# OverLordGoldDragon/ssqueezepy

Hardware: AMD Instinct MI355X
Metric: ssq_cwt transforms/sec (N=160k, 300 scales, f32) (higher is better)
Workload: dtype f32; 1 GPU; ssq_cwt('gmw'), N=160000, 300 log scales (nv=32), float32, two-chirp+noise; algo=blockzoom+tiles, tile_kernel=float64 tile, unordered ds_add_f64, column pair per lane (tile3_kernel)

## Files before the change

include/ssq_hip.h:

```cpp
#ifndef SSQ_HIP_H
#define SSQ_HIP_H

#include <stdint.h>

#ifdef __cplusplus
extern "C" {
#endif

#define SSQ_F32 0
#define SSQ_F64 1

#define SSQ_GRID_LOG 0
#define SSQ_GRID_LOG_PIECEWISE 1
#define SSQ_GRID_LIN 2

#define SSQ_PAD_NONE (-1)
#define SSQ_PAD_ZERO 0
#define SSQ_PAD_REFLECT 1
#define SSQ_PAD_SYMMETRIC 2
#define SSQ_PAD_REPLICATE 3
#define SSQ_PAD_WRAP 4

int         ssq_version(void);
const char* ssq_build_sha(void);
// ... 145 lines not shown
    const int32_t* generic_rows;
    int64_t        n_generic;
} ssq_cwt_blocks_desc;

int  ssq_cwt_plan_set_blocks(ssq_cwt_plan* plan, const ssq_cwt_blocks_desc* desc);

typedef struct {
    int32_t        n_segs;
    const int32_t* segs;
    int32_t        n_steps;
    const int32_t* rows;
    const void*    wtab;
    int64_t        n_phases;
    const void*    tbank;
    int64_t        n_tbank;
    int32_t        n_irows;
    const int64_t* irows;
    int32_t        n_classes;
    const int64_t* classes;
    int64_t        u_total;
    int64_t        n_items_tile[5];
    int32_t        reserved;
} ssq_cwt_tiles_desc;

int  ssq_cwt_plan_set_tiles(ssq_cwt_plan* plan, const ssq_cwt_tiles_desc* desc);

int  ssq_cwt_plan_timing(ssq_cwt_plan* plan, int enable, double* stage_ms, int64_t* signals);

int  ssq_cwt_plan_group(const ssq_cwt_plan* plan);

int64_t ssq_cwt_plan_tiles_done(ssq_cwt_plan* plan, void* stream);
int  ssq_cwt_plan_tile_cols(const ssq_cwt_plan* plan);
int  ssq_cwt_plan_tile_kernel(const ssq_cwt_plan* plan);
int  ssq_cwt_plan_tile_counters(ssq_cwt_plan* plan, unsigned long long* out, int n, void* stream);

int  ssq_cwt_plan_set_bin_dump(ssq_cwt_plan* plan, unsigned short* kmap);

int  ssq_cwt_tile_rows_per_step(void);

int64_t ssq_cwt_plan_bytes(const ssq_cwt_plan* plan);
const char* ssq_cwt_plan_algo(const ssq_cwt_plan* plan);

typedef struct ssq_stft_plan ssq_stft_plan;

typedef struct {
    int      dtype;
    int      padtype;
    int64_t  n;
    int64_t  n_fft;
    int64_t  hop_len;
    int      modulated;
    const void* window;
    const void* diff_window;
    int64_t  max_batch;
} ssq_stft_desc;

int  ssq_stft_plan_create(ssq_stft_plan** plan, const ssq_stft_desc* desc);
void ssq_stft_plan_destroy(ssq_stft_plan* plan);
int  ssq_stft_plan_set_ssq(ssq_stft_plan* plan, const void* Sfs, int grid,
                           const double* params, const void* cst, int cst_f64,
                           int flipud, double gamma);
int  ssq_stft_plan_shape(const ssq_stft_plan* plan, int64_t* rows, int64_t* n_hops);
const char* ssq_stft_plan_algo(const ssq_stft_plan* plan);
int  ssq_stft_execute(ssq_stft_plan* plan, const void* x, int64_t batch, void* Sx,
                      void* dSx, void* Tx, void* w, void* stream);
int  ssq_stft_adjoint(ssq_stft_plan* plan, const void* gSx, const void* gdSx, void* gx,
// ... 7 lines not shown
```

ssqueezepy_amd/_cwt.py:

```python
import ctypes
import logging
import os
import numpy as np
import torch

from . import _lib
from ._lib import check, F32, F64, CwtDesc, CwtBlocksDesc, CwtTilesDesc
from . import algos
from ._bank import banded_bank, support_hull
from ._blocks import plan_blocks, L_MIN
from ._tiles import plan_tiles, RSUB as _tiles_rsub
from .padding import pad_geometry, PADTYPES
from .scales import process_scales, _process_fs_and_t
from .wavelets import Wavelet

WARN = lambda msg: logging.warning("WARNING: %s" % msg)

__all__ = ['cwt', 'cwt_higher_order', 'CwtPlan', 'get_cwt_plan', 'clear_plan_cache']

_TDT = {'float32': torch.float32, 'float64': torch.float64}
_CDT = {'float32': torch.complex64, 'float64': torch.complex128}


class CwtPlan():
# ... 137 lines not shown
        d.n_classes, d.classes = len(classes), classes.ctypes.data
        d.u_total = tp['u_total']
        d.reserved = _tiles_rsub
        for slot in range(5):
            d.n_items_tile[slot] = n_items_tile[slot]
        check(self.lib.ssq_cwt_plan_set_tiles(self._h, ctypes.byref(d)))
        self.tile_rows = int(tp['interp_rows'].sum())
        self.tile_plan = {k: tp[k] for k in ('lgR', 'interp_rows', 'classes')}

    def __del__(self):
        h = getattr(self, '_h', None)
        if h is not None and h.value:
            try:
                self.lib.ssq_cwt_plan_destroy(h)
            except Exception:
                pass
            self._h = None

    @property
    def algo(self):
        return self.lib.ssq_cwt_plan_algo(self._h).decode()

    def tiles_done(self):
        return int(self.lib.ssq_cwt_plan_tiles_done(self._h, algos.stream()))

    @property
    def tile_cols(self):
        return int(self.lib.ssq_cwt_plan_tile_cols(self._h))

    @property
    def tile_kernel(self):
        return int(self.lib.ssq_cwt_plan_tile_kernel(self._h))

    def set_bin_dump(self, kmap):
        if kmap is not None and (kmap.element_size() != 2 or kmap.numel() < self.max_batch * self.na * self.N
                                 or not kmap.is_contiguous()):
            raise ValueError("bin dump: a contiguous 2-byte tensor of max_batch * na * N elements is needed")
        check(self.lib.ssq_cwt_plan_set_bin_dump(self._h, kmap.data_ptr() if kmap is not None else None))
        self._kdump = kmap

    def tiles_per_signal(self, N):
        if not self.tile_cols:
            return 0
        lead = (self.n1 & 1) if self.tile_kernel == 3 else 0
        return -(-(int(N) + lead) // self.tile_cols)

    @property
    def device_bytes(self):
        return int(self.lib.ssq_cwt_plan_bytes(self._h))

    @property
    def group(self):
        return int(self.lib.ssq_cwt_plan_group(self._h))

    def timing(self, enable=-1):
        ms = (ctypes.c_double * 4)()
        n = ctypes.c_int64()
        check(self.lib.ssq_cwt_plan_timing(self._h, int(enable), ms, ctypes.byref(n)))
        return list(ms), int(n.value)

    def set_ssq(self, grid, params, const, flipud, gamma):
        const = np.asarray(const)
        if const.size != self.na:
            const = np.full(self.na, float(const)).astype(self.dtype)
        const = const.reshape(-1)
        c64 = int(self.dtype == 'float32' and const.dtype == np.float64)
# ... 263 lines not shown
```

ssqueezepy_amd/_lib.py:

```python
import ctypes
import os
from ctypes import (c_int, c_int64, c_double, c_void_p, c_char_p, POINTER,
                    Structure)

HERE = os.path.dirname(os.path.abspath(__file__))
LIB_PATH = os.environ.get('SSQ_HIP_LIB') or os.path.join(HERE, 'libssq_hip.so')

F32, F64 = 0, 1
GRID_LOG, GRID_LOG_PIECEWISE, GRID_LIN = 0, 1, 2
PAD = {None: -1, 'zero': 0, 'reflect': 1, 'symmetric': 2, 'replicate': 3,
       'wrap': 4}


class SsqError(RuntimeError):
    pass


class CwtDesc(Structure):
    _fields_ = [('dtype', c_int), ('padtype', c_int), ('n', c_int64),
                ('m', c_int64), ('n1', c_int64), ('na', c_int64),
                ('bank', c_void_p), ('band_off', c_void_p), ('band_lo', c_void_p),
                ('dt', c_double), ('row_scale', c_void_p), ('max_batch', c_int64),
                ('algo', c_int)]

# ... 71 lines not shown
    'ssq_colsum_adjoint': (c_int, [c_int, c_void_p, c_void_p, c_void_p, c_int64, c_int64,
                                   c_int64, c_void_p]),
    'ssq_band_colsum_batch': (c_int, [c_int, c_void_p, c_void_p, c_void_p, c_int, c_int64,
                                      c_void_p, c_int64, c_int64, c_int64, c_void_p]),
    'ssq_band_colsum_adjoint': (c_int, [c_int, c_void_p, c_void_p, c_void_p, c_int, c_int64,
                                        c_void_p, c_int64, c_int64, c_int64, c_void_p]),
    'ssq_ridge_energy': (c_int, [c_int, c_int, c_void_p, c_void_p, c_int64, c_int64, c_void_p]),
    'ssq_ridge_neglog': (c_int, [c_int, c_void_p, c_void_p, c_double, c_int64, c_int64, c_void_p]),
    'ssq_ridge_track': (c_int, [c_int, c_int, c_void_p, c_void_p, c_void_p, c_double, c_double,
                                c_int64, c_int64, c_void_p, c_void_p]),
    'ssq_ridge_clear': (c_int, [c_int, c_void_p, c_void_p, c_double, c_void_p, c_int64, c_int64,
                                c_void_p]),
    'ssq_ridge_neglog_batch': (c_int, [c_int, c_void_p, c_void_p, c_double, c_int64, c_int64, c_int64,
                                       c_void_p]),
    'ssq_ridge_track_batch': (c_int, [c_int, c_int, c_void_p, c_void_p, c_void_p, c_double, c_double,
                                      c_int64, c_int64, c_void_p, c_int64, c_void_p]),
    'ssq_ridge_clear_batch': (c_int, [c_int, c_void_p, c_void_p, c_double, c_void_p, c_int64, c_int64,
                                      c_int64, c_void_p]),
    'ssq_cwt_plan_create': (c_int, [POINTER(c_void_p), POINTER(CwtDesc)]),
    'ssq_cwt_plan_destroy': (None, [c_void_p]),
    'ssq_cwt_plan_set_ssq': (c_int, [c_void_p, c_int, POINTER(c_double), c_void_p,
                                     c_int, c_int, c_double]),
    'ssq_cwt_execute': (c_int, [c_void_p, c_void_p, c_int64, c_void_p, c_void_p,
                                c_void_p, c_void_p, c_int, c_void_p]),
    'ssq_cwt_plan_set_blocks': (c_int, [c_void_p, POINTER(CwtBlocksDesc)]),
    'ssq_cwt_plan_set_tiles': (c_int, [c_void_p, POINTER(CwtTilesDesc)]),
    'ssq_cwt_plan_timing': (c_int, [c_void_p, c_int, POINTER(c_double), POINTER(c_int64)]),
    'ssq_cwt_plan_group': (c_int, [c_void_p]),
    'ssq_cwt_plan_bytes': (c_int64, [c_void_p]),
    'ssq_cwt_plan_algo': (c_char_p, [c_void_p]),
    'ssq_cwt_plan_tiles_done': (c_int64, [c_void_p, c_void_p]),
    'ssq_cwt_plan_tile_cols': (c_int, [c_void_p]),
    'ssq_cwt_plan_tile_kernel': (c_int, [c_void_p]),
    'ssq_cwt_plan_tile_counters': (c_int, [c_void_p, c_void_p, c_int, c_void_p]),
    'ssq_cwt_plan_set_bin_dump': (c_int, [c_void_p, c_void_p]),
    'ssq_build_sha': (c_char_p, []),
    'ssq_cwt_tile_rows_per_step': (c_int, []),
    'ssq_stft_plan_create': (c_int, [POINTER(c_void_p), POINTER(StftDesc)]),
    'ssq_stft_plan_destroy': (None, [c_void_p]),
    'ssq_stft_plan_set_ssq': (c_int, [c_void_p, c_void_p, c_int, POINTER(c_double),
                                      c_void_p, c_int, c_int, c_double]),
    'ssq_stft_plan_shape': (c_int, [c_void_p, POINTER(c_int64), POINTER(c_int64)]),
    'ssq_stft_plan_algo': (c_char_p, [c_void_p]),
    'ssq_stft_execute': (c_int, [c_void_p, c_void_p, c_int64, c_void_p, c_void_p,
                                 c_void_p, c_void_p, c_void_p]),
    'ssq_stft_adjoint': (c_int, [c_void_p, c_void_p, c_void_p, c_void_p, c_int64, c_void_p]),
}

EXPORTS = tuple(_PROTOS)
_lib = None


ABI_VERSION = 107


def load(build_if_missing=True):
    global _lib
    if _lib is not None:
        return _lib
    if not os.path.isfile(LIB_PATH):
        if not build_if_missing:
            raise SsqError("libssq_hip.so not found at %s; run "
                           "`python -m ssqueezepy_amd.build`" % LIB_PATH)
        from .build import build
        build(verbose=False)
    try:
        lib = ctypes.CDLL(LIB_PATH)
    except OSError as e:
        raise SsqError("cannot load %s: %s. The ssqueezepy_amd compute path has no "
                       "CPU fallback; it needs the ROCm runtime (libamdhip64, "
                       "librocfft)." % (LIB_PATH, e))
    lib.ssq_version.restype, lib.ssq_version.argtypes = c_int, []
    if lib.ssq_version() < ABI_VERSION:
        raise SsqError("%s is an older build (ABI %d, this package needs %d); rebuild with "
                       "`python -m ssqueezepy_amd.build`"
                       % (LIB_PATH, lib.ssq_version(), ABI_VERSION))
    for name, (res, args) in _PROTOS.items():
        fn = getattr(lib, name)
        fn.restype = res
        fn.argtypes = args
    _lib = lib
    return lib


def check(rc):
    if rc != 0:
# ... 11 lines not shown
```

ssqueezepy_amd/csrc/ssq_cwt.hip:

```cpp
#include "ssq_common.h"
#include "ssq_fft.h"
#include "ssq_blocks.h"
#include "ssq_tiles.h"
#include <algorithm>
#include <map>
#include <string>
#include <vector>

namespace ssq {

#include "ssq_point_math.inl"

template <typename T>
__global__ __launch_bounds__(256) void bank_multiply_kernel(
    const T* __restrict__ xh,
    const T* __restrict__ bank, const int64_t* __restrict__ band_off,
    const int32_t* __restrict__ band_lo,
    T* __restrict__ prod,
    int64_t M, const int32_t* __restrict__ rowlist, int64_t row0, int nplanes, double h, T inv_dt) {
    const int64_t r = blockIdx.y;
    const int64_t i = rowlist[row0 + r];
    const int64_t lo = band_lo[i];
    const int64_t off = band_off[i];
    const int64_t len = band_off[i + 1] - off;
// ... 278 lines not shown
    if (stage_ms) for (int t = 0; t < 4; ++t) stage_ms[t] = pl->stage_ms[t];
    if (signals) *signals = pl->timed_signals;
    if (enable >= 0) {
        pl->timing = enable != 0;
        for (int t = 0; t < 4; ++t) pl->stage_ms[t] = 0;
        pl->timed_signals = 0;
    }
    return 0;
}

int ssq_cwt_plan_set_bin_dump(ssq_cwt_plan* pl, unsigned short* kmap) {
    SSQ_REQUIRE(pl, "ssq_cwt_plan_set_bin_dump: null plan");
    std::lock_guard<std::mutex> lock(pl->order.mu);
    pl->kdump = kmap;
    return 0;
}

int ssq_cwt_plan_group(const ssq_cwt_plan* pl) { return pl ? pl->group : 0; }
int ssq_cwt_tile_rows_per_step(void) { return ssq::tile_rows_per_step(); }
int64_t ssq_cwt_plan_tiles_done(ssq_cwt_plan* pl, void* stream) {
    if (!pl || !pl->tile) return 0;
    return pl->tile->tiles_done(as_stream(stream));
}
int ssq_cwt_plan_tile_cols(const ssq_cwt_plan* pl) { return (pl && pl->tile) ? pl->tile->tile_cols() : 0; }
int ssq_cwt_plan_tile_counters(ssq_cwt_plan* pl, unsigned long long* out, int n, void* stream) {
    SSQ_REQUIRE(pl && out && n >= 0 && n <= 512, "ssq_cwt_plan_tile_counters: bad arguments");
    memset(out, 0, (size_t)n * 8);
    if (!pl->tile || !pl->tile->counters) return 0;
    SSQ_CHECK_HIP(hipStreamSynchronize(as_stream(stream)));
    SSQ_CHECK_HIP(hipMemcpy(out, pl->tile->counters, (size_t)n * 8, hipMemcpyDeviceToHost));
    return 0;
}
int ssq_cwt_plan_tile_kernel(const ssq_cwt_plan* pl) { return (pl && pl->tile) ? pl->tile->tile_kernel() : 0; }
int64_t ssq_cwt_plan_bytes(const ssq_cwt_plan* pl) { return pl ? pl->bytes : 0; }
const char* ssq_cwt_plan_algo(const ssq_cwt_plan* pl) { return pl ? pl->algo.c_str() : ""; }

}

template <typename T>
static int cwt_execute_t(ssq_cwt_plan* pl, const void* x, int64_t batch, void* Wx, void* dWx,
                         void* Tx, void* w, int rpadded, hipStream_t stream) {
    const ssq_cwt_desc& d = pl->d;
    const int64_t M = d.m, N = d.n, na = d.na;
    const int64_t out_cols = rpadded ? M : N;
    const bool deriv = dWx || Tx || w;
    const int nplanes = deriv ? 2 : 1;
    const double h = (2.0 * 3.141592653589793) / (double)M;
    const T inv_dt = T(1) / (T)d.dt;
    if (pl->timing && pl->tev.size() < 2) {
        for (int t = 0; t < 2; ++t) { hipEvent_t e; SSQ_CHECK_HIP(hipEventCreate(&e)); pl->tev.push_back(e); }
    }
    if (pl->timing) (void)hipEventRecord(pl->tev[0], stream);

    const T* xsrc = (const T*)x;
    if (d.padtype != SSQ_PAD_NONE) {
        int rc = ssq_pad_signal(d.dtype, x, pl->xp, batch, N, d.n1, M - N - d.n1, d.padtype, stream);
        if (rc) return rc;
        xsrc = (const T*)pl->xp;
    } else {
        SSQ_CHECK_HIP(hipMemcpyAsync(pl->xp, x, (size_t)batch * M * sizeof(T), hipMemcpyDeviceToDevice, stream));
        xsrc = (const T*)pl->xp;
    }
    if (batch == d.max_batch) {
        int rc = pl->fwd.execute((void*)xsrc, pl->xh, stream);
        if (rc) return rc;
    } else {
// ... 172 lines not shown
```

ssqueezepy_amd/csrc/ssq_cwt_tiles.hip:

```cpp
#include "ssq_common.h"
#include "ssq_tiles.h"
#include <algorithm>
#include <cmath>

namespace ssq {

int tile_rows_per_step() { return TILE_G; }

struct ItemTable {
    int n = 0;
    std::vector<int32_t> rec;
    std::vector<int32_t> cls;
    std::vector<int32_t> woff;
    bool ok = true;
};
static ItemTable pack_items(const TileSeg* sg, int nsegs, const TileRow* rw, int nsteps, int64_t M, int64_t N, int rpi,
                            bool woff_in_record) {
    ItemTable t;
    t.n = nsteps * TILE_G / rpi;
    t.rec.assign((size_t)t.n * 8, 0); t.cls.assign((size_t)t.n, 0); t.woff.assign((size_t)t.n, 0);
    for (int i = 0; i < nsegs; ++i) {
        const int64_t L = (int64_t)M >> sg[i].lgR;
        if (sg[i].kind && (sg[i].wtab_off >= (woff_in_record ? 16384 : 65536) || sg[i].sig_stride % L)) t.ok = false;
        for (int s = 0; s < sg[i].nsteps * TILE_G / rpi; ++s) {
// ... 197 lines not shown
        if ((rc = up(&items2, t2.rec.data(), t2.rec.size() * 4))) return rc;
        if ((rc = up((void**)&wave_first2, waves.data(), waves.size() * 4))) return rc;
        tile3_ok = false;
        if (cols2 == 32) {
            ItemTable t3 = pack_items(sg, nsegs, rw, nsteps, M, N, 4, true);
            std::vector<int32_t> dealt;
            tile3_ok = deal_item_lists(t3, TILE3_NW, 0.45f, 0.65f, dealt, waves);
            n_items3 = t3.n;
            if ((rc = up(&items3, dealt.data(), dealt.size() * 4))) return rc;
            if ((rc = up((void**)&wave_first3, waves.data(), waves.size() * 4))) return rc;
            for (int i = 0; i < nsegs; ++i) if (sg[i].kind && sg[i].lgR < 2) tile3_ok = false;
        }
    }
    {
        const TileSeg* sg = reinterpret_cast<const TileSeg*>(d.segs);
        const float* src = reinterpret_cast<const float*>(d.wtab);
        std::vector<float> w((size_t)16 * d.n_phases, 0.f);
        std::vector<char> done((size_t)d.n_phases, 0);
        for (int i = 0; i < nsegs; ++i) {
            if (sg[i].kind != 1) continue;
            const int64_t R = (int64_t)1 << sg[i].lgR, o = sg[i].wtab_off;
            SSQ_REQUIRE(o >= 0 && o + R <= d.n_phases, "tile segment %d: weights outside the table", i);
            if (done[(size_t)o]) continue;
            done[(size_t)o] = 1;
            for (int64_t ph = 0; ph < R; ++ph)
                for (int t = 0; t < 4; ++t)
                    for (int k = 0; k < 4; ++k)
                        w[(size_t)(16 * o + (t * R + ph) * 4 + k)] = src[(size_t)(16 * (o + ph) + 4 * t + k)];
        }
        if ((rc = up(&wtab, w.data(), (size_t)64 * d.n_phases))) return rc;
    }
    if ((rc = up(&tbank, d.tbank, (size_t)4 * d.n_tbank))) return rc;
    cls.resize(d.n_classes);
    const bool own_fft = !(getenv("SSQ_DEBUG_TILE_FFT") && !strcmp(getenv("SSQ_DEBUG_TILE_FFT"), "rocfft"));
    int64_t y_entries = 0;
    for (int c = 0; c < d.n_classes; ++c) {
        cls[c] = {d.classes[4 * c], d.classes[4 * c + 1], d.classes[4 * c + 2], 0, 0, 0};
        SSQ_REQUIRE(cls[c].L >= 2 && (cls[c].L & (cls[c].L - 1)) == 0 && cls[c].nrows >= 1, "bad tile class %d", c);
        lmax = std::max(lmax, cls[c].L);
        int lg = 0;
        while (((int64_t)1 << lg) < cls[c].L) ++lg;
        if (own_fft && lg >= 13 && lg <= 22) {
            cls[c].B = 1 << ((lg + 1) / 2); cls[c].A = 1 << (lg / 2);
            y_entries += (int64_t)group * cls[c].nrows * cls[c].L;
        } else if (own_fft && lg >= 6 && lg <= 12) {
            cls[c].B = 1;
        }
    }
    std::vector<TileIRow> hi;
    hi.reserve((size_t)n_irows);
    for (int pass = 0; pass < 2; ++pass)
        for (int c = 0; c < d.n_classes; ++c) {
            if ((cls[c].A > 0 || cls[c].B > 0) != (pass == 0)) continue;
            if (pass == 1 && n_irows_fft == 0) first_irow_fft = (int)hi.size();
            cls[c].first = (int)hi.size();
            for (int r = 0; r < n_irows; ++r) {
                const int64_t* q = d.irows + 8 * r;
                if ((int)q[6] != c) continue;
                SSQ_REQUIRE(q[4] == cls[c].L && q[2] >= 1 && 2 * q[2] <= q[4]
                            && q[1] >= 0 && q[1] + q[2] <= M / 2 + 1 && q[5] >= 0 && q[5] + q[2] <= d.n_tbank
                            && q[7] >= 0 && q[7] < cls[c].nrows, "bad tile row %d", r);
                hi.push_back({(int32_t)q[0], (int32_t)q[1], (int32_t)q[2], (int32_t)q[3], (int32_t)q[4], (int32_t)q[5],
                              (int32_t)((int64_t)group * cls[c].upre + q[7] * cls[c].L), (int32_t)(cls[c].nrows * cls[c].L)});
            }
            SSQ_REQUIRE((int64_t)hi.size() - cls[c].first == cls[c].nrows, "tile class %d: %lld rows listed, %lld declared",
                        c, (long long)((int64_t)hi.size() - cls[c].first), (long long)cls[c].nrows);
            if (pass == 1) n_irows_fft += (int)cls[c].nrows;
        }
    SSQ_REQUIRE((int)hi.size() == n_irows, "tile rows of unknown classes");
    if ((rc = up((void**)&irows, hi.data(), sizeof(TileIRow) * n_irows))) return rc;
    if (own_fft) {
        SSQ_CHECK_HIP(hipMalloc(&Y, (size_t)8 * std::max<int64_t>(y_entries, 1))); bytes += 8 * y_entries;
        std::vector<float> tw;
        for (int s = 0; s < 7; ++s) {
            const int Lp = 64 << s;
            ftw_off[s] = (int64_t)tw.size() / 2;
            for (int q = 0; q < Lp; ++q) {
                const double a = 6.283185307179586 * (double)q / (double)Lp;
                tw.push_back((float)std::cos(a)); tw.push_back((float)std::sin(a));
            }
        }
        if ((rc = up(&ftw, tw.data(), tw.size() * 4))) return rc;
    }
    SSQ_CHECK_HIP(hipMalloc(&U, (size_t)8 * (group * u_total + 4 * lmax))); bytes += 8 * (group * u_total + 4 * lmax);
    SSQ_CHECK_HIP(hipMemset(U, 0, (size_t)8 * (group * u_total + 4 * lmax)));
    SSQ_CHECK_HIP(hipMalloc((void**)&counters, 4096));
    SSQ_CHECK_HIP(hipMemset(counters, 0, 4096));
    for (size_t c = 0; c < cls.size(); ++c) {
        FftPlan fp;
        if (!cls[c].A && !cls[c].B) {
            rc = fp.create(1, SSQ_F32, (size_t)cls[c].L, (size_t)(group * cls[c].nrows), 1.0);
            if (rc) return rc;
            bytes += (int64_t)fp.work_bytes;
        }
        ffts.push_back(fp);
    }
    for (int t = 0; t < 5; ++t) n_items_tile[t] = d.n_items_tile[t];
    SSQ_CHECK_HIP(hipStreamCreateWithFlags(&side, hipStreamNonBlocking));
    SSQ_CHECK_HIP(hipEventCreateWithFlags(&ev_fork, hipEventDisableTiming));
    SSQ_CHECK_HIP(hipEventCreateWithFlags(&ev_join, hipEventDisableTiming));
    return 0;
}

void TilePlan::destroy() {
    if (side) { (void)hipStreamSynchronize(side); (void)hipStreamDestroy(side); side = nullptr; }
// ... 36 lines not shown
        return run_ordered(sig, nsig, Wx, dWx, Tx, kidx, cst, cst0, sp, stream);
    default:
        set_error("na = %lld: no tile kernel can run in this mode (the executor asks usable() first)", (long long)na);
        return -1;
    }
}

TileWalkArgs TilePlan::walk_args(const void* items, const int32_t* waves, int sig, int nsig, float* Wx, float* dWx,
                                 float* Tx, const unsigned short* kidx, const void* cst, float cst0,
                                 const SsqParams& sp, unsigned short* kdump) const {
    TileWalkArgs A{};
    A.items = reinterpret_cast<const int*>(items); A.waves = reinterpret_cast<const int4*>(waves);
    A.wtab = (const float4*)wtab; A.U = (const float2*)U; A.cst = cst;
    A.Wx = (float2*)Wx; A.dWx = (float2*)dWx; A.Tx = (float2*)Tx; A.kidx = kidx; A.kdump = kdump;
    A.N = N; A.na = na; A.n1 = (int)n1; A.mmask = (int)(M - 1);
    A.lgM = 0; while (((int64_t)1 << A.lgM) < M) ++A.lgM;
    A.sig0 = sig; A.nsig = nsig; A.carry = 0; A.xcd = 0;
    A.inv_m = 1.0f / (float)M; A.theta_scale = (float)(6.283185307179586 / ((double)M * dt)); A.cst0 = cst0;
    A.counters = counters; A.gamma = sp.gamma;
    return A;
}

int TilePlan::walk_grid(int64_t ntx, int cols, int per_cu, TileWalkArgs& A) const {
    const int64_t cap = (int64_t)ncu * per_cu;
    const int64_t q = std::max<int64_t>(1, ((int64_t)1 << lgr_max2) / cols);
    const int64_t G = ntx <= cap ? ntx : std::max<int64_t>(q, cap / q * q);
    const char* ce = getenv("SSQ_DEBUG_TILE2_CARRY");
    A.carry = (!(ce && atoi(ce) == 0) && ntx > G && ntx % q == 0) ? 1 : 0;
    const char* xe = getenv("SSQ_DEBUG_TILE2_XCD");
    A.xcd = !(xe && atoi(xe) == 0) && G >= 16;
    return (int)G;
}

int64_t TilePlan::tiles_done(hipStream_t stream) {
    unsigned long long v = 0;
    if (!counters) return 0;
    if (hipStreamSynchronize(stream) != hipSuccess) return -1;
    if (hipMemcpy(&v, counters, 8, hipMemcpyDeviceToHost) != hipSuccess) return -1;
    return (int64_t)v;
}

}
```

ssqueezepy_amd/csrc/ssq_kernels.hip:

```cpp
#include "ssq_common.h"
#include <cstdlib>
#include <mutex>
#include <string>

namespace ssq {

static thread_local std::string g_last_error;

void set_error(const char* fmt, ...) {
    char buf[1024];
    va_list ap;
    va_start(ap, fmt);
    vsnprintf(buf, sizeof(buf), fmt, ap);
    va_end(ap);
    g_last_error = buf;
}

#include "ssq_point_math.inl"

template <typename T, bool CST64>
__device__ __forceinline__ void weighted_add(T& o_re, T& o_im, T c, T d, const void* cst, int64_t i) {
    if constexpr (CST64 && sizeof(T) == 4) {
        double w = ((const double*)cst)[i];
        o_re = (T)((double)o_re + (double)c * w);
// ... 604 lines not shown
        case SSQ_PAD_REPLICATE: return t < 0 ? 0 : n - 1;
        case SSQ_PAD_WRAP: { int64_t m = t % n; if (m < 0) m += n; return m; }
        default: return -1;
    }
}

template <typename T>
__global__ __launch_bounds__(256) void pad_kernel(const T* __restrict__ x, T* __restrict__ out,
                                                  int64_t n, int64_t n1, int64_t m, int padtype,
                                                  int64_t total) {
    for (int64_t t = (int64_t)blockIdx.x * blockDim.x + threadIdx.x; t < total;
         t += (int64_t)gridDim.x * blockDim.x) {
        int64_t b = t / m, p = t % m;
        int64_t s = pad_source(p - n1, n, padtype);
        out[t] = s < 0 ? T(0) : x[b * n + s];
    }
}

static inline unsigned stream_grid(int64_t total, int block = 256) {
    int64_t g = (total + block - 1) / block;
    const int64_t cap = 256 * 8 * 4;
    return (unsigned)(g < 1 ? 1 : (g > cap ? cap : g));
}

}

using namespace ssq;

extern "C" __attribute__((weak)) const char ssq_build_sha_value[] = "unknown";

extern "C" {

const char* ssq_build_sha(void) { return ssq_build_sha_value; }
int ssq_version(void) { return 107; }
const char* ssq_last_error(void) { return g_last_error.c_str(); }

int ssq_device_count(int* count) {
    SSQ_REQUIRE(count, "ssq_device_count: null pointer");
    SSQ_CHECK_HIP(hipGetDeviceCount(count));
    return 0;
}
int ssq_set_device(int device) { SSQ_CHECK_HIP(hipSetDevice(device)); return 0; }

int ssq_device_info(int device, char* name, int len, int* cus, int64_t* hbm_bytes) {
    hipDeviceProp_t prop;
    SSQ_CHECK_HIP(hipGetDeviceProperties(&prop, device));
    if (name && len > 0) { strncpy(name, prop.gcnArchName, len - 1); name[len - 1] = 0; }
    if (cus) *cus = prop.multiProcessorCount;
    if (hbm_bytes) *hbm_bytes = (int64_t)prop.totalGlobalMem;
    return 0;
}

int ssq_malloc(void** ptr, int64_t bytes) {
    SSQ_REQUIRE(ptr && bytes >= 0, "ssq_malloc: bad arguments");
    SSQ_CHECK_HIP(hipMalloc(ptr, (size_t)(bytes > 0 ? bytes : 1)));
    return 0;
}
int ssq_free(void* ptr) { SSQ_CHECK_HIP(hipFree(ptr)); return 0; }
int ssq_memcpy_h2d(void* dst, const void* src, int64_t bytes, void* stream) {
    SSQ_CHECK_HIP(hipMemcpyAsync(dst, src, (size_t)bytes, hipMemcpyHostToDevice, as_stream(stream)));
    return 0;
}
int ssq_memcpy_d2h(void* dst, const void* src, int64_t bytes, void* stream) {
    SSQ_CHECK_HIP(hipMemcpyAsync(dst, src, (size_t)bytes, hipMemcpyDeviceToHost, as_stream(stream)));
    return 0;
}
int ssq_memset(void* dst, int value, int64_t bytes, void* stream) {
// ... 151 lines not shown
```

ssqueezepy_amd/csrc/ssq_tile_fft.hip:

```cpp
#include "ssq_common.h"
#include "ssq_tiles.h"
#include "ssq_ldsfft.h"
#include <algorithm>
#include <cmath>

namespace ssq {

__global__ __launch_bounds__(256) void tile_spectra_kernel(const float2* __restrict__ xh_all,
                                                           int64_t xh_stride, int sig0,
                                                           const TileIRow* __restrict__ irows,
                                                           const float* __restrict__ tbank,
                                                           float2* __restrict__ U) {
    const TileIRow r = irows[blockIdx.y];
    const int s = blockIdx.z;
    const float2* xh = xh_all + (int64_t)(sig0 + s) * xh_stride;
    float2* u = U + r.ubase + (int64_t)s * r.sig_stride;
    const int half = r.L >> 1;
    for (int p = blockIdx.x * blockDim.x + threadIdx.x; p < r.L; p += gridDim.x * blockDim.x) {
        const int kk = p < half ? p : p - r.L;
        const int t = r.kc + kk - r.lo;
        float2 z = make_float2(0.f, 0.f);
        if (t >= 0 && t < r.K) {
            const float2 x = xh[r.lo + t];
            const float b = tbank[r.tb_off + t];
// ... 181 lines not shown
    for (int it = 0; it < PPT; ++it) {
        const int idx = tid + it * NT, q = idx & (L - 1), g = idx >> LGL;
        const int j = block * G + g;
        if (j < npairs) {
            const int jr = j % E.nrows, js = j / E.nrows;
            const TileIRow row = E.irows[jr];
            E.U[row.ubase + (int64_t)js * row.sig_stride + q] = buf[g * (L + 1) + q];
        }
    }
}

struct TileSmallArgs {
    TileFftArgs E[7];
    int first_block[8];
    int npairs[7], slot[7];
    int ncls;
};
__global__ __launch_bounds__(NT) void tilefft_small_kernel(TileSmallArgs A) {
    __shared__ c32 buf[D_POINTS + 64];
    int b = (int)blockIdx.x, c = 0;
    while (c + 1 < A.ncls && b >= A.first_block[c + 1]) ++c;
    b -= A.first_block[c];
    switch (A.slot[c]) {
        case 0: tilefft_small_body<64, 64, 8, 8, 1>(A.E[c], A.npairs[c], b, buf); break;
        case 1: tilefft_small_body<128, 32, 16, 8, 1>(A.E[c], A.npairs[c], b, buf); break;
        case 2: tilefft_small_body<256, 16, 16, 16, 1>(A.E[c], A.npairs[c], b, buf); break;
        case 3: tilefft_small_body<512, 8, 8, 8, 8>(A.E[c], A.npairs[c], b, buf); break;
        case 4: tilefft_small_body<1024, 4, 16, 8, 8>(A.E[c], A.npairs[c], b, buf); break;
        case 5: tilefft_small_body<2048, 2, 16, 16, 8>(A.E[c], A.npairs[c], b, buf); break;
        default: tilefft_small_body<4096, 1, 16, 16, 16>(A.E[c], A.npairs[c], b, buf); break;
    }
}

int TilePlan::spectra(int sig, int nsig, const void* xh_all, hipStream_t stream) {
    {
        TileSmallArgs S;
        S.ncls = 0; S.first_block[0] = 0;
        for (int want = 6; want >= 0; --want)
            for (size_t c = 0; c < cls.size() && S.ncls < 7; ++c) {
                if (cls[c].A || !cls[c].B) continue;
                int sl = 0;
                while ((64 << sl) < cls[c].L) ++sl;
                if (sl != want) continue;
                TileFftArgs& E = S.E[S.ncls];
                E.xh = (const c32*)xh_all; E.xh_stride = M / 2 + 1; E.sig0 = sig;
                E.irows = irows + cls[c].first; E.tbank = (const float*)tbank;
                E.Y = nullptr; E.U = (c32*)U;
                E.A = 0; E.B = 0; E.L = (int)cls[c].L; E.nrows = (int)cls[c].nrows; E.G2 = 0; E.inv_l = 0.f; E.nyq = 0;
                E.ftw1 = (const c32*)ftw + ftw_off[sl]; E.ftw2 = nullptr;
                const int G = D_POINTS / (int)cls[c].L, npairs = E.nrows * nsig;
                S.npairs[S.ncls] = npairs; S.slot[S.ncls] = sl;
                S.first_block[S.ncls + 1] = S.first_block[S.ncls] + (npairs + G - 1) / G;
                ++S.ncls;
            }
        if (S.ncls) {
            hipLaunchKernelGGL(tilefft_small_kernel, dim3((unsigned)S.first_block[S.ncls]), dim3(NT), 0, stream, S);
            SSQ_LAUNCH_CHECK();
        }
    }
    {
        TileFourArgs F1, F2;
        F1.ncls = 0; F1.first_block[0] = 0; F2.first_block[0] = 0;
        int64_t y_off = 0;
        for (size_t c = 0; c < cls.size() && F1.ncls < 10; ++c) {
            if (!cls[c].A) continue;
            const int k = F1.ncls;
            TileFftArgs E;
            E.xh = (const c32*)xh_all; E.xh_stride = M / 2 + 1; E.sig0 = sig;
            E.irows = irows + cls[c].first; E.tbank = (const float*)tbank;
            E.Y = (c32*)Y + y_off; E.U = (c32*)U;
            y_off += (int64_t)group * cls[c].nrows * cls[c].L;
            E.A = cls[c].A; E.B = cls[c].B; E.L = (int)cls[c].L; E.nrows = (int)cls[c].nrows;
            E.G2 = D_POINTS / E.A;
            E.inv_l = 1.0f / (float)cls[c].L; E.nyq = 0;
            int sa = 0, sb = 0;
            while ((64 << sa) < E.A) ++sa;
            while ((64 << sb) < E.B) ++sb;
            E.ftw1 = (const c32*)ftw + ftw_off[sb]; E.ftw2 = (const c32*)ftw + ftw_off[sa];
            F1.E[k] = E; F2.E[k] = E;
            F1.slot[k] = sb; F2.slot[k] = sa;
            F1.nx[k] = E.A / (D_POINTS / E.B);
            F2.nx[k] = E.B / E.G2;
            F1.first_block[k + 1] = F1.first_block[k] + F1.nx[k] * E.nrows * nsig;
            F2.first_block[k + 1] = F2.first_block[k] + F2.nx[k] * E.nrows * nsig;
            ++F1.ncls;
        }
        F2.ncls = F1.ncls;
        if (F1.ncls) {
            hipLaunchKernelGGL(tilefft_four_kernel<1>, dim3((unsigned)F1.first_block[F1.ncls]), dim3(NT), 0, stream, F1);
// ... 87 lines not shown
```

ssqueezepy_amd/csrc/ssq_tiles.h:

```cpp
#pragma once
#include "ssq_common.h"
#include "ssq_fft.h"
#include <type_traits>
#include <vector>

namespace ssq {

struct TileSeg {
    int32_t kind;
    int32_t first;
    int32_t nsteps;
    int32_t lgR;
    int32_t wtab_off;
    int32_t sig_stride;
    int32_t lmask;
    int32_t cls_base;
};
struct TileRow {
    int32_t row;
    int32_t ubase;
    int32_t kc;
    float   theta;
};
struct TileIRow {
// ... 32 lines not shown
    unsigned short* kdump;
    int64_t N, na;
    int pad0_, n1, mmask, lgM, sig0, nsig, pad1_;
    int carry;
    int xcd;
    float inv_m, theta_scale, cst0;
    unsigned long long* counters;
    double gamma;
};

struct TilePlan {
    int64_t M = 0, N = 0, n1 = 0, na = 0;
    int group = 1;
    double dt = 1.0;
    int nsegs = 0, nsteps = 0, n_irows = 0;
    int64_t u_total = 0, lmax = 0;
    int ncu = 0;
    int4* steps = nullptr;
    int2* rows = nullptr;
    TileIRow* irows = nullptr;
    void* wtab = nullptr; void* tbank = nullptr;
    void* U = nullptr;
    unsigned long long* counters = nullptr;
    void* items2 = nullptr; int32_t* wave_first2 = nullptr;
    int n_items2 = 0, cols2 = 32;
    int lgr_max2 = 0;
    bool tile2_ok = false;
    void* items3 = nullptr; int32_t* wave_first3 = nullptr;
    int n_items3 = 0;
    bool tile3_ok = false;
    int tile_kernel() const;
    int tile_cols() const;
    bool usable() const { return tile_kernel() != 0; }
    struct Cls { int64_t L, nrows, upre; int A, B, first; };
    std::vector<Cls> cls;
    std::vector<FftPlan> ffts;
    int n_irows_fft = 0, first_irow_fft = 0;
    void* Y = nullptr;
    void* ftw = nullptr;
    int64_t ftw_off[7] = {0, 0, 0, 0, 0, 0, 0};
    int64_t n_items_tile[5] = {0, 0, 0, 0, 0};
    std::vector<unsigned char> class_need;
    hipStream_t side = nullptr; hipEvent_t ev_fork = nullptr, ev_join = nullptr;

    int create(const ssq_cwt_tiles_desc& d, int64_t M, int64_t N, int64_t n1, int64_t na, int group,
               double dt, int64_t& bytes);
    void destroy();
    int spectra(int sig, int nsig, const void* xh_all, hipStream_t stream);
    int run(int sig, int nsig, float* Wx, float* dWx, float* Tx, const unsigned short* kidx,
            const void* cst, float cst0, const SsqParams& sp, hipStream_t stream, unsigned short* kdump = nullptr);
    int run_ordered(int sig, int nsig, float* Wx, float* dWx, float* Tx, const unsigned short* kidx,
                    const void* cst, float cst0, const SsqParams& sp, hipStream_t stream);
    int run_f64(int sig, int nsig, float* Wx, float* dWx, float* Tx, const unsigned short* kidx,
                const void* cst, float cst0, const SsqParams& sp, hipStream_t stream, unsigned short* kdump);
    int run_pair(int sig, int nsig, float* Wx, float* dWx, float* Tx, const unsigned short* kidx,
                 const void* cst, float cst0, const SsqParams& sp, hipStream_t stream, unsigned short* kdump);
    TileWalkArgs walk_args(const void* items, const int32_t* waves, int sig, int nsig, float* Wx, float* dWx, float* Tx,
                           const unsigned short* kidx, const void* cst, float cst0, const SsqParams& sp,
                           unsigned short* kdump) const;
    int walk_grid(int64_t ntx, int cols, int per_cu, TileWalkArgs& A) const;
    int64_t tiles_done(hipStream_t stream);
};

template <bool BIN_DUMP = true, class F>
int tile_dispatch(const SsqParams& sp, bool store_d, bool store_k, F&& f) {
    using std::integral_constant;
    using K0 = integral_constant<int, 0>; using K1 = integral_constant<int, 1>; using K2 = integral_constant<int, 2>;
    auto by_weights = [&](auto grid, auto d) -> int {
// ... 27 lines not shown
```

Baseline: 3769 transforms/s.

## Add single-kernel tile FFT route for 8K-64K length classes

Adds a one-kernel tile FFT path for classes with FFT length 2^13 to 2^16 (up to four classes). It does a radix-C pre-pass with twiddles while loading inputs, then a 4096-point LDS inverse FFT per block, and writes the output directly. This replaces the four-step path, which needed an intermediate Y buffer in global memory and two passes. The cost is high register and LDS pressure from 1024-thread blocks plus a register/LDS stash for the C=8 case. It also adds a routes query API for diagnostics.

```diff
diff --git a/include/ssq_hip.h b/include/ssq_hip.h
--- a/include/ssq_hip.h
+++ b/include/ssq_hip.h
@@ -201,6 +201,7 @@
 int64_t ssq_cwt_plan_tiles_done(ssq_cwt_plan* plan, void* stream);
 int  ssq_cwt_plan_tile_cols(const ssq_cwt_plan* plan);
 int  ssq_cwt_plan_tile_kernel(const ssq_cwt_plan* plan);
+int  ssq_cwt_plan_tile_fft_routes(const ssq_cwt_plan* plan, int64_t out[5]);
 int  ssq_cwt_plan_tile_counters(ssq_cwt_plan* plan, unsigned long long* out, int n, void* stream);
 
 int  ssq_cwt_plan_set_bin_dump(ssq_cwt_plan* plan, unsigned short* kmap);
diff --git a/ssqueezepy_amd/_cwt.py b/ssqueezepy_amd/_cwt.py
--- a/ssqueezepy_amd/_cwt.py
+++ b/ssqueezepy_amd/_cwt.py
@@ -193,6 +193,11 @@
     def tile_kernel(self):
         return int(self.lib.ssq_cwt_plan_tile_kernel(self._h))
 
+    def tile_fft_routes(self):
+        out = (ctypes.c_int64 * 5)()
+        check(self.lib.ssq_cwt_plan_tile_fft_routes(self._h, out))
+        return dict(zip(('one_kernel', 'four_step', 'small', 'rocfft', 'y_bytes'), (int(v) for v in out)))
+
     def set_bin_dump(self, kmap):
         if kmap is not None and (kmap.element_size() != 2 or kmap.numel() < self.max_batch * self.na * self.N
                                  or not kmap.is_contiguous()):
diff --git a/ssqueezepy_amd/_lib.py b/ssqueezepy_amd/_lib.py
--- a/ssqueezepy_amd/_lib.py
+++ b/ssqueezepy_amd/_lib.py
@@ -127,6 +127,7 @@
     'ssq_cwt_plan_tiles_done': (c_int64, [c_void_p, c_void_p]),
     'ssq_cwt_plan_tile_cols': (c_int, [c_void_p]),
     'ssq_cwt_plan_tile_kernel': (c_int, [c_void_p]),
+    'ssq_cwt_plan_tile_fft_routes': (c_int, [c_void_p, POINTER(c_int64)]),
     'ssq_cwt_plan_tile_counters': (c_int, [c_void_p, c_void_p, c_int, c_void_p]),
     'ssq_cwt_plan_set_bin_dump': (c_int, [c_void_p, c_void_p]),
     'ssq_build_sha': (c_char_p, []),
@@ -146,7 +147,7 @@
 _lib = None
 
 
-ABI_VERSION = 107
+ABI_VERSION = 108
 
 
 def load(build_if_missing=True):
diff --git a/ssqueezepy_amd/csrc/ssq_cwt.hip b/ssqueezepy_amd/csrc/ssq_cwt.hip
--- a/ssqueezepy_amd/csrc/ssq_cwt.hip
+++ b/ssqueezepy_amd/csrc/ssq_cwt.hip
@@ -334,6 +334,12 @@
     return 0;
 }
 int ssq_cwt_plan_tile_kernel(const ssq_cwt_plan* pl) { return (pl && pl->tile) ? pl->tile->tile_kernel() : 0; }
+int ssq_cwt_plan_tile_fft_routes(const ssq_cwt_plan* pl, int64_t* out) {
+    SSQ_REQUIRE(pl && out, "ssq_cwt_plan_tile_fft_routes: bad arguments");
+    memset(out, 0, 5 * sizeof(int64_t));
+    if (pl->tile) pl->tile->routes(out);
+    return 0;
+}
 int64_t ssq_cwt_plan_bytes(const ssq_cwt_plan* pl) { return pl ? pl->bytes : 0; }
 const char* ssq_cwt_plan_algo(const ssq_cwt_plan* pl) { return pl ? pl->algo.c_str() : ""; }
 
diff --git a/ssqueezepy_amd/csrc/ssq_cwt_tiles.hip b/ssqueezepy_amd/csrc/ssq_cwt_tiles.hip
--- a/ssqueezepy_amd/csrc/ssq_cwt_tiles.hip
+++ b/ssqueezepy_amd/csrc/ssq_cwt_tiles.hip
@@ -253,15 +253,21 @@
     }
     if ((rc = up(&tbank, d.tbank, (size_t)4 * d.n_tbank))) return rc;
     cls.resize(d.n_classes);
-    const bool own_fft = !(getenv("SSQ_DEBUG_TILE_FFT") && !strcmp(getenv("SSQ_DEBUG_TILE_FFT"), "rocfft"));
+    const char* fft_env = getenv("SSQ_DEBUG_TILE_FFT");
+    const bool own_fft = !(fft_env && !strcmp(fft_env, "rocfft"));
+    const bool one_fft = own_fft && !(fft_env && !strcmp(fft_env, "fourstep"));
     int64_t y_entries = 0;
+    int n_one = 0;
     for (int c = 0; c < d.n_classes; ++c) {
         cls[c] = {d.classes[4 * c], d.classes[4 * c + 1], d.classes[4 * c + 2], 0, 0, 0};
         SSQ_REQUIRE(cls[c].L >= 2 && (cls[c].L & (cls[c].L - 1)) == 0 && cls[c].nrows >= 1, "bad tile class %d", c);
         lmax = std::max(lmax, cls[c].L);
         int lg = 0;
         while (((int64_t)1 << lg) < cls[c].L) ++lg;
-        if (own_fft && lg >= 13 && lg <= 22) {
+        if (one_fft && lg >= 13 && lg <= 16 && n_one < 4) {
+            cls[c].B = 1; cls[c].C = 1 << (lg - 13);
+            ++n_one;
+        } else if (own_fft && lg >= 13 && lg <= 22) {
             cls[c].B = 1 << ((lg + 1) / 2); cls[c].A = 1 << (lg / 2);
             y_entries += (int64_t)group * cls[c].nrows * cls[c].L;
         } else if (own_fft && lg >= 6 && lg <= 12) {
@@ -291,7 +297,8 @@
     SSQ_REQUIRE((int)hi.size() == n_irows, "tile rows of unknown classes");
     if ((rc = up((void**)&irows, hi.data(), sizeof(TileIRow) * n_irows))) return rc;
     if (own_fft) {
-        SSQ_CHECK_HIP(hipMalloc(&Y, (size_t)8 * std::max<int64_t>(y_entries, 1))); bytes += 8 * y_entries;
+        y_bytes = 8 * y_entries;
+        if (y_bytes) { SSQ_CHECK_HIP(hipMalloc(&Y, (size_t)y_bytes)); bytes += y_bytes; }
         std::vector<float> tw;
         for (int s = 0; s < 7; ++s) {
             const int Lp = 64 << s;
@@ -394,6 +401,12 @@
     return (int)G;
 }
 
+void TilePlan::routes(int64_t out[5]) const {
+    for (int i = 0; i < 5; ++i) out[i] = 0;
+    for (const Cls& c : cls) ++out[c.C ? 0 : c.A ? 1 : c.B ? 2 : 3];
+    out[4] = y_bytes;
+}
+
 int64_t TilePlan::tiles_done(hipStream_t stream) {
     unsigned long long v = 0;
     if (!counters) return 0;
diff --git a/ssqueezepy_amd/csrc/ssq_kernels.hip b/ssqueezepy_amd/csrc/ssq_kernels.hip
--- a/ssqueezepy_amd/csrc/ssq_kernels.hip
+++ b/ssqueezepy_amd/csrc/ssq_kernels.hip
@@ -660,7 +660,7 @@
 extern "C" {
 
 const char* ssq_build_sha(void) { return ssq_build_sha_value; }
-int ssq_version(void) { return 107; }
+int ssq_version(void) { return 108; }
 const char* ssq_last_error(void) { return g_last_error.c_str(); }
 
 int ssq_device_count(int* count) {
diff --git a/ssqueezepy_amd/csrc/ssq_tile_fft.hip b/ssqueezepy_amd/csrc/ssq_tile_fft.hip
--- a/ssqueezepy_amd/csrc/ssq_tile_fft.hip
+++ b/ssqueezepy_amd/csrc/ssq_tile_fft.hip
@@ -237,13 +237,130 @@
     }
 }
 
+constexpr int ONE_NT = 1024;
+constexpr int ONE_S = 4096;
+constexpr int ONE_STASH = 3;
+constexpr int ONE_LDS = 4 * ONE_S + 32 + ONE_STASH * ONE_NT;
+
+template <int C>
+__device__ __forceinline__ void tilefft_one_body(const TileFftArgs& E, int npairs, int block, c32* lds) {
+    constexpr int G = C >= 4 ? 4 : C, ROUNDS = C / G;
+    constexpr int TG = 256 * G, UPW = ONE_NT / TG;
+    constexpr int NK = ONE_S / TG;
+    constexpr int H = ONE_S * C;
+    constexpr int CS = ONE_S + (G > 1 ? 32 / G : 0);
+    static_assert(NK * G == PPT, "a round is 16 points per work-item");
+    const int tid = threadIdx.x, ui = tid / TG, lt = tid % TG;
+    const int pair = UPW == 1 ? ((block >> 4) << 3) + (block & 7) : (block * UPW + ui) >> 1;
+    const int par = UPW == 1 ? (block >> 3) & 1 : (block * UPW + ui) & 1;
+    const bool live = pair < npairs;
+    const int jr = live ? pair % E.nrows : 0, js = live ? pair / E.nrows : 0;
+    const TileIRow row = E.irows[jr];
+    const c32* xh = E.xh + (int64_t)(E.sig0 + js) * E.xh_stride + row.lo;
+    const float* tb = E.tbank + row.tb_off;
+    const int kk0 = row.lo - row.kc;
+    const float inv_h = 2.0f * E.inv_l;
+    c32* ub = lds + ui * (G * ONE_S + 32);
+    c32 zh[NK][G];
+    c32* stash = lds + 4 * ONE_S + 32 + tid;
+    auto inputs = [&](auto odd) {
+#pragma unroll
+        for (int j = 0; j < NK; ++j) {
+            const int k1 = lt + j * TG;
+            c32 z[C];
+#pragma unroll
+            for (int k2 = 0; k2 < C; ++k2) {
+                const int t = (k1 + ONE_S * k2 - kk0) & (H - 1), kk = kk0 + t;
+                const bool in = live && t < row.K && kk >= -H && kk < H;
+                const unsigned tc = t < row.K ? t : 0;
+                const c32 X = xh[tc];
+                const float b = tb[tc];
+                c32 v = {in ? X.x * b : 0.f, in ? X.y * b : 0.f};
+                if constexpr (decltype(odd)::value) {
+                    const float rev = (float)kk * E.inv_l;
+                    const c32 tw = {__builtin_amdgcn_cosf(rev), __builtin_amdgcn_sinf(rev)};
+                    v = cmul_v(v, tw);
+                }
+                z[k2] = v;
+            }
+            if constexpr (C == 8) Dft<8>::run(z);
+            else if constexpr (C == 4) Dft<4>::run(z);
+            else if constexpr (C == 2) dft2(z[0], z[1]);
+#pragma unroll
+            for (int q2 = 1; q2 < C; ++q2) {
+                const float rev = (float)(k1 * q2) * inv_h;
+                const c32 tw = {__builtin_amdgcn_cosf(rev), __builtin_amdgcn_sinf(rev)};
+                z[q2] = cmul_v(z[q2], tw);
+            }
+#pragma unroll
+            for (int c = 0; c < G; ++c) {
+                if constexpr (C == 1) zh[j][c] = z[c];
+                else ub[c * CS + k1] = z[c];
+                if constexpr (ROUNDS == 2) {
+                    if (j * G + c < ONE_STASH) stash[(j * G + c) * ONE_NT] = z[G + c];
+                    else zh[j][c] = z[G + c];
+                }
+            }
+            if ((j + 1) * C % 16 == 0) SSQ_SCHED_FENCE();
+        }
+    };
+    if (par) inputs(std::true_type{}); else inputs(std::false_type{});
+    c32* u_out = E.U + row.ubase + (int64_t)js * row.sig_stride + par;
+    const int g = lt % G, u = lt / G;
+#pragma unroll
+    for (int r = 0; r < ROUNDS; ++r) {
+        c32 v[PPT];
+        if constexpr (C == 1) {
+#pragma unroll
+            for (int j = 0; j < NK; ++j) v[j] = zh[j][0];
+        } else {
+            if (r) {
+                __syncthreads();
+#pragma unroll
+                for (int j = 0; j < NK; ++j)
+#pragma unroll
+                    for (int c = 0; c < G; ++c) ub[c * CS + lt + j * TG] = j * G + c < ONE_STASH ? stash[(j * G + c) * ONE_NT] : zh[j][c];
+            }
+            __syncthreads();
+#pragma unroll
+            for (int t = 0; t < PPT; ++t) v[t] = ub[g * CS + u + 256 * t];
+        }
+        lds_ifft<ONE_S, G, 16, 16, 16, ROUNDS == 1, false, 1, TG>(v, ub, E.ftw1, lt);
+        SSQ_SCHED_FENCE();
+        if (live) {
+            const int q2 = r * G + g;
+#pragma unroll
+            for (int k = 0; k < PPT; ++k) u_out[(unsigned)(2 * (q2 + C * (u + 256 * k)))] = v[k];
+        }
+    }
+}
+
+struct TileOneArgs {
+    TileFftArgs E[4];
+    int first_block[5];
+    int npairs[4], lgc[4];
+    int ncls;
+};
+__global__ __launch_bounds__(ONE_NT) void tilefft_one_kernel(TileOneArgs A) {
+    __shared__ c32 buf[ONE_LDS];
+    int b = (int)blockIdx.x, c = 0;
+    while (c + 1 < A.ncls && b >= A.first_block[c + 1]) ++c;
+    b -= A.first_block[c];
+    switch (A.lgc[c]) {
+        case 3: tilefft_one_body<8>(A.E[c], A.npairs[c], b, buf); break;
+        case 2: tilefft_one_body<4>(A.E[c], A.npairs[c], b, buf); break;
+        case 1: tilefft_one_body<2>(A.E[c], A.npairs[c], b, buf); break;
+        default: tilefft_one_body<1>(A.E[c], A.npairs[c], b, buf); break;
+    }
+}
+
 int TilePlan::spectra(int sig, int nsig, const void* xh_all, hipStream_t stream) {
     {
         TileSmallArgs S;
         S.ncls = 0; S.first_block[0] = 0;
         for (int want = 6; want >= 0; --want)
             for (size_t c = 0; c < cls.size() && S.ncls < 7; ++c) {
-                if (cls[c].A || !cls[c].B) continue;
+                if (cls[c].A || !cls[c].B || cls[c].C) continue;
                 int sl = 0;
                 while ((64 << sl) < cls[c].L) ++sl;
                 if (sl != want) continue;
@@ -260,6 +377,32 @@
             }
         if (S.ncls) {
             hipLaunchKernelGGL(tilefft_small_kernel, dim3((unsigned)S.first_block[S.ncls]), dim3(NT), 0, stream, S);
+            SSQ_LAUNCH_CHECK();
+        }
+    }
+    {
+        TileOneArgs O;
+        O.ncls = 0; O.first_block[0] = 0;
+        for (size_t c = 0; c < cls.size() && O.ncls < 4; ++c) {
+            if (!cls[c].C) continue;
+            const int k = O.ncls;
+            TileFftArgs& E = O.E[k];
+            E.xh = (const c32*)xh_all; E.xh_stride = M / 2 + 1; E.sig0 = sig;
+            E.irows = irows + cls[c].first; E.tbank = (const float*)tbank;
+            E.Y = nullptr; E.U = (c32*)U;
+            E.A = 0; E.B = 0; E.L = (int)cls[c].L; E.nrows = (int)cls[c].nrows; E.G2 = 0; E.nyq = 0;
+            E.inv_l = 1.0f / (float)cls[c].L;
+            E.ftw1 = (const c32*)ftw + ftw_off[6]; E.ftw2 = nullptr;
+            int lgc = 0;
+            while ((1 << lgc) < cls[c].C) ++lgc;
+            const int npairs = E.nrows * nsig;
+            const int upw = cls[c].C >= 4 ? 1 : cls[c].C == 2 ? 2 : 4;
+            O.npairs[k] = npairs; O.lgc[k] = lgc;
+            O.first_block[k + 1] = O.first_block[k] + (upw == 1 ? 16 * ((npairs + 7) / 8) : (2 * npairs + upw - 1) / upw);
+            ++O.ncls;
+        }
+        if (O.ncls) {
+            hipLaunchKernelGGL(tilefft_one_kernel, dim3((unsigned)O.first_block[O.ncls]), dim3(ONE_NT), 0, stream, O);
             SSQ_LAUNCH_CHECK();
         }
     }
diff --git a/ssqueezepy_amd/csrc/ssq_tiles.h b/ssqueezepy_amd/csrc/ssq_tiles.h
--- a/ssqueezepy_amd/csrc/ssq_tiles.h
+++ b/ssqueezepy_amd/csrc/ssq_tiles.h
@@ -88,8 +88,10 @@
     int tile_kernel() const;
     int tile_cols() const;
     bool usable() const { return tile_kernel() != 0; }
-    struct Cls { int64_t L, nrows, upre; int A, B, first; };
+    struct Cls { int64_t L, nrows, upre; int A, B, first; int C = 0; };
     std::vector<Cls> cls;
+    int64_t y_bytes = 0;
+    void routes(int64_t out[5]) const;
     std::vector<FftPlan> ffts;
     int n_irows_fft = 0, first_irow_fft = 0;
     void* Y = nullptr;
```

New measurement: 3718 transforms/s. -1.4%, worse.
